# ppwwyyxx/OpenPano

Measured on NVIDIA H100. Metric: Mpixels/sec SIFT+match+blend, higher is better.
Workload: dtype f32

## Files before the change

openpano_b200/csrc/blend.cu:

```cuda
#include "common.cuh"
#include "blur_tile.cuh"
#include <math.h>
#include <string.h>
#include <vector>
#include <algorithm>
#include <climits>
#include <memory>

struct BlendImg {
  union {
    const float* rgb;
    const unsigned char* pix;
  };
  int w, h;
  int x0, y0, x1, y1;
  double hi[9];
  long long roi_off;
  long long plane;
  long long mask_off;
  int rw, rh, pitch;
  int channels;
};

template <class Src> __device__ __forceinline__ Src blend_src(const BlendImg& im, const float* lut);
template <> __device__ __forceinline__ SrcF32 blend_src<SrcF32>(const BlendImg& im, const float*) { return SrcF32{im.rgb}; }
template <> __device__ __forceinline__ SrcRgb8 blend_src<SrcRgb8>(const BlendImg& im, const float* lut) {
  return SrcRgb8{im.pix, lut, im.channels};
}
template <> __device__ __forceinline__ SrcPix8 blend_src<SrcPix8>(const BlendImg& im, const float* lut) {
  return SrcPix8{im.pix, lut, im.channels, (size_t)im.w * im.h};
}

struct BlendGeom {
  int projection;
  double res_x, res_y, min_x, min_y;
  const double* col_sin;
  const double* col_cos;
  const double* row_tan;
};

__device__ __forceinline__ void coor_func(const BlendImg& im, const BlendGeom& g, int tx, int ty, double* ox, double* oy) {
  double cx = (double)tx * g.res_x + g.min_x;
  double cy = (double)ty * g.res_y + g.min_y;
  double hx, hy, hz;
  if (g.projection == PANO_PROJ_FLAT) { hx = cx; hy = cy; hz = 1.0; }
  else if (g.projection == PANO_PROJ_CYLINDRICAL) { hx = g.col_sin[tx]; hy = cy; hz = g.col_cos[tx]; }
  else { hx = g.col_sin[tx]; hy = g.row_tan[ty]; hz = g.col_cos[tx]; }
  double rx = im.hi[0] * hx + im.hi[1] * hy + im.hi[2] * hz;
  double ry = im.hi[3] * hx + im.hi[4] * hy + im.hi[5] * hz;
  double rz = im.hi[6] * hx + im.hi[7] * hy + im.hi[8] * hz;
  if (rz < 0) { *ox = -10; *oy = -10; return; }
  double denom = 1.0 / rz;
  *ox = rx * denom + im.w * 0.5;
  *oy = ry * denom + im.h * 0.5;
}

#define TILE_LIST_CAP 64
struct TileList { int n; unsigned short idx[TILE_LIST_CAP]; };

__device__ __forceinline__ void build_tile_list(const BlendImg* __restrict__ imgs, int n, int j0, int i0, int j1, int i1,
                                                TileList* tl) {
  const int tid = threadIdx.y * blockDim.x + threadIdx.x;
  if (tid < 32) {
    int cnt = 0;
    for (int base = 0; base < n; base += 32) {
      const int k = base + tid;
      bool hit = false;
      if (k < n) {
        const BlendImg& im = imgs[k];
        hit = im.y0 <= i1 && im.y1 >= i0 && im.x0 <= j1 && im.x1 >= j0;
      }
      const unsigned bal = __ballot_sync(0xffffffffu, hit);
      if (hit) {
        const int slot = cnt + __popc(bal & ((1u << tid) - 1));
        if (slot < TILE_LIST_CAP) tl->idx[slot] = (unsigned short)k;
      }
      cnt += __popc(bal);
    }
    if (tid == 0) tl->n = (cnt <= TILE_LIST_CAP && n <= 65535) ? cnt : -1;
  }
  __syncthreads();
}


template <class Src>
__device__ __forceinline__ void linear_add_px(const BlendImg* __restrict__ imgs, int n, const TileList& tl,
                                              const BlendGeom& g, int lazy, int ordered, const float* lut, int i, int j,
                                              float& s0, float& s1, float& s2, float& wsum) {
  const int nl = tl.n < 0 ? n : tl.n;
  for (int q = 0; q < nl; ++q) {
    const BlendImg& im = imgs[tl.n < 0 ? q : (int)tl.idx[q]];
    bool in = lazy ? (i >= im.y0 && i < im.y1 && j >= im.x0 && j < im.x1)
                   : (i >= im.y0 && i <= im.y1 && j >= im.x0 && j <= im.x1);
    if (!in) continue;
    double x, y;
    coor_func(im, g, j, i, &x, &y);
    if (x < 0 || x >= im.w || y < 0 || y >= im.h) continue;
    float r = (float)y, c = (float)x;
    float c0, c1, c2;
    if (!interpolate_rgb(blend_src<Src>(im, lut), im.w, im.h, r, c, &c0, &c1, &c2)) continue;
    if (c0 < 0) continue;
    float w = (float)(0.5 - fabs((double)(c / (float)im.w) - 0.5));
    if (!ordered) w = (float)((double)w * (0.5 - fabs((double)(r / (float)im.h) - 0.5)));
    s0 += c0 * w; s1 += c1 * w; s2 += c2 * w;
    wsum += w;
  }
}

__device__ __forceinline__ void linear_resolve_px(int lazy, float s0, float s1, float s2, float wsum, float* p) {
  if (lazy) {
    if (wsum != 0.f) { p[0] = s0 / wsum; p[1] = s1 / wsum; p[2] = s2 / wsum; }
    else { p[0] = -1.f; p[1] = -1.f; p[2] = -1.f; }
  } else {
    if (wsum > 0) {
      float inv = (float)(1.0 / (double)wsum);
      p[0] = s0 * inv; p[1] = s1 * inv; p[2] = s2 * inv;
    } else { p[0] = -1.f; p[1] = -1.f; p[2] = -1.f; }
  }
}

template <class Src>
__global__ void k_linear_blend(const BlendImg* __restrict__ imgs, int n, BlendGeom g, int lazy, int ordered,
                               float* __restrict__ out, int tw, int row0, int row1) {
  __shared__ TileList tl;
  __shared__ float lut[Src::kLut ? 256 : 1];
  if constexpr (Src::kLut) build_rgb8_lut(lut, threadIdx.y * blockDim.x + threadIdx.x);
  {
    const int tj0 = blockIdx.x * blockDim.x, ti0 = row0 + blockIdx.y * blockDim.y;
    build_tile_list(imgs, n, tj0, ti0, tj0 + blockDim.x - 1, ti0 + blockDim.y - 1, &tl);
  }
  int j = blockIdx.x * blockDim.x + threadIdx.x;
  int i = row0 + blockIdx.y * blockDim.y + threadIdx.y;
  if (j >= tw || i >= row1) return;
  float s0 = 0.f, s1 = 0.f, s2 = 0.f, wsum = 0.f;
  linear_add_px<Src>(imgs, n, tl, g, lazy, ordered, lut, i, j, s0, s1, s2, wsum);
  linear_resolve_px(lazy, s0, s1, s2, wsum, out + ((size_t)(i - row0) * tw + j) * 3);
}

template <class Src>
__global__ void k_linear_accumulate(const BlendImg* __restrict__ imgs, int n, BlendGeom g, int lazy, int ordered,
                                    float* __restrict__ sum, float* __restrict__ wsum, int tw, int rx0, int ry0, int rx1,
                                    int ry1) {
  __shared__ TileList tl;
  __shared__ float lut[Src::kLut ? 256 : 1];
  if constexpr (Src::kLut) build_rgb8_lut(lut, threadIdx.y * blockDim.x + threadIdx.x);
  const int tj0 = rx0 + blockIdx.x * blockDim.x, ti0 = ry0 + blockIdx.y * blockDim.y;
  build_tile_list(imgs, n, tj0, ti0, tj0 + blockDim.x - 1, ti0 + blockDim.y - 1, &tl);
  const int j = tj0 + threadIdx.x, i = ti0 + threadIdx.y;
  if (tl.n == 0 || j >= rx1 || i >= ry1) return;
  const size_t t = (size_t)i * tw + j;
  float* p = sum + t * 3;
  float s0 = p[0], s1 = p[1], s2 = p[2], ws = wsum[t];
  linear_add_px<Src>(imgs, n, tl, g, lazy, ordered, lut, i, j, s0, s1, s2, ws);
  p[0] = s0; p[1] = s1; p[2] = s2;
  wsum[t] = ws;
}

__global__ void k_linear_resolve(const float* sum, const float* __restrict__ wsum, float* out, size_t n_px, int lazy) {
  const size_t t = (size_t)blockIdx.x * blockDim.x + threadIdx.x;
  if (t >= n_px) return;
  const float* p = sum + t * 3;
  linear_resolve_px(lazy, p[0], p[1], p[2], wsum[t], out + t * 3);
}

template <class Src>
__global__ void k_mb_first_level(const BlendImg* __restrict__ imgs, BlendGeom g, float* __restrict__ cur,
                                 unsigned char* __restrict__ mask) {
  __shared__ float lut[Src::kLut ? 256 : 1];
  if constexpr (Src::kLut) {
    build_rgb8_lut(lut, threadIdx.y * blockDim.x + threadIdx.x);
    __syncthreads();
  }
  const BlendImg& im = imgs[blockIdx.z];
  int j = blockIdx.x * blockDim.x + threadIdx.x;
  int i = blockIdx.y * blockDim.y + threadIdx.y;
  if (j >= im.rw || i >= im.rh) return;
  double x, y;
  coor_func(im, g, j + im.x0, i + im.y0, &x, &y);
  float c0, c1, c2;
  bool ok = interpolate_rgb(blend_src<Src>(im, lut), im.w, im.h, (float)y, (float)x, &c0, &c1, &c2);
  if (ok && fminf(c0, fminf(c1, c2)) < 0) ok = false;
  const size_t o = (size_t)i * im.pitch + j;
  float* p = cur + im.roi_off + o;
  float ww = 0.f;
  if (!ok) { c0 = 0.f; c1 = 0.f; c2 = 0.f; }
  else {
    double ox = x / im.w - 0.5, oy = y / im.h - 0.5;
    double wd = (0.5 - fabs(ox)) * (0.5 - fabs(oy));
    if (wd < 0.0) wd = 0.0;
    ww = (float)(wd + 1e-6);
  }
  p[0] = c0; p[im.plane] = c1; p[2 * im.plane] = c2; p[3 * im.plane] = ww;
  mask[im.mask_off + o] = ok ? 0 : 1;
}

__global__ void k_mb_weight_argmax(const BlendImg* __restrict__ imgs, int n, float* __restrict__ cur, int tw,
                                   int row0, int row1) {
  __shared__ TileList tl;
  {
    const int tj0 = blockIdx.x * blockDim.x, ti0 = row0 + blockIdx.y * blockDim.y;
    build_tile_list(imgs, n, tj0, ti0, tj0 + blockDim.x - 1, ti0 + blockDim.y - 1, &tl);
  }
  int j = blockIdx.x * blockDim.x + threadIdx.x;
  int i = row0 + blockIdx.y * blockDim.y + threadIdx.y;
  if (j >= tw || i >= row1) return;
  const int nl = tl.n < 0 ? n : tl.n;
  float mx = 0.f;
  int best = -1;
  for (int q = 0; q < nl; ++q) {
    const BlendImg& im = imgs[tl.n < 0 ? q : (int)tl.idx[q]];
    if (i >= im.y0 && i <= im.y1 && j >= im.x0 && j <= im.x1) {
      const float w = __ldg(cur + im.roi_off + 3 * im.plane + (size_t)(i - im.y0) * im.pitch + (j - im.x0));
      if (w > mx) { mx = w; best = q; }
    }
  }
  for (int q = 0; q < nl; ++q) {
    const BlendImg& im = imgs[tl.n < 0 ? q : (int)tl.idx[q]];
    if (i >= im.y0 && i <= im.y1 && j >= im.x0 && j <= im.x1)
      cur[im.roi_off + 3 * im.plane + (size_t)(i - im.y0) * im.pitch + (j - im.x0)] = q == best ? 1.f : 0.f;
  }
}

struct BlurTaps { int center; float taps[64]; };
struct MbPlane { long long off; int w, h, pitch, pad; };

template <int C>
__global__ void __launch_bounds__(BT_THREADS, 4)
k_mb_blur_tma(const MbPlane* __restrict__ planes, const int2* __restrict__ span, int n_planes, int n_tiles,
              const TmaDesc* __restrict__ maps, float* __restrict__ dst, const __grid_constant__ BlurTaps bt) {
  extern __shared__ __align__(128) float smem[];
  __shared__ __align__(8) uint64_t s_bar[2];
  __shared__ BlurTile s_tile[2];
  constexpr int RX = (C + 3) & ~3;
  constexpr int GW = BT_W + 2 * RX, GH = BT_H + 2 * C;
  constexpr int GSZ = (GH * GW + 31) & ~31;
  float* grey0 = smem;
  float* colbuf = smem + 2 * GSZ;
  float* outT = colbuf + BLUR_COLBUF_FLOATS(C);
// ... 134 lines not shown
  if (is_last && touched) {
    v0 = v0 < 1.0f ? v0 : 1.0f; v0 = v0 > 0.f ? v0 : 0.f;
    v1 = v1 < 1.0f ? v1 : 1.0f; v1 = v1 > 0.f ? v1 : 0.f;
    v2 = v2 < 1.0f ? v2 : 1.0f; v2 = v2 > 0.f ? v2 : 0.f;
    dirty = true;
  }
  if (dirty) { p[0] = v0; p[1] = v1; p[2] = v2; }
  if (first || touched) tmask[t] = touched ? 1 : 0;
}

__global__ void k_fill(float* __restrict__ p, size_t n, float v) {
  size_t i = (size_t)blockIdx.x * blockDim.x + threadIdx.x;
  if (i < n) p[i] = v;
}


struct BlendJob {
  std::vector<BlendImg> imgs;
  BlendGeom g;
  int tw = 0, th = 0;
  long long roi_floats = 0;
  long long mask_bytes = 0;
  int max_rw = 0, max_rh = 0;
  std::vector<BlurTaps> level_taps;
  int halo = 0;
  bool strip = false;
  int clip0 = INT_MIN, clip1 = INT_MAX;
  std::vector<double> tab;
  size_t ncol = 0, nrow = 0;
};

struct BlendDev {
  DevBuf<BlendImg> d_imgs;
  DevBuf<double> d_tab;
  DevBuf<float> d_cur, d_next;
  DevBuf<unsigned char> d_mask, d_tmask;
  DevBuf<MbPlane> d_planes;
  DevBuf<int2> d_span;
  DevBuf<TmaDesc> d_maps;
  std::vector<int> centers;
  int n_planes = 0, n_tiles = 0;
  int wrow0 = 0, wrow1 = 0;
};

template <int C>
static cudaError_t launch_mb_blur_tma(pano_ctx* ctx, int grid, const MbPlane* planes, const int2* span, int n_planes,
                                      int n_tiles, const TmaDesc* maps, float* dst, const BlurTaps& bt) {
  constexpr int RX = (C + 3) & ~3, GW = BT_W + 2 * RX, GH = BT_H + 2 * C, GSZ = (GH * GW + 31) & ~31;
  const size_t smem = (size_t)(2 * GSZ + BLUR_COLBUF_FLOATS(C) + BT_H * (BT_W + 1)) * sizeof(float);
  cudaError_t e = cudaFuncSetAttribute(k_mb_blur_tma<C>, cudaFuncAttributeMaxDynamicSharedMemorySize, (int)smem);
  if (e != cudaSuccess) return e;
  k_mb_blur_tma<C><<<grid, BT_THREADS, smem, ctx->stream>>>(planes, span, n_planes, n_tiles, maps, dst, bt);
  return cudaGetLastError();
}

static int blend_plan(pano_ctx* ctx, int n, const pano_blend_image* imgs, const pano_blend_geom* g, int bands,
                      const pano_params* p, int ow, int oh, int row0, int row1, bool need_src, BlendJob* job,
                      const unsigned char* const* pix = nullptr, const int* channels = nullptr) {
  for (int level = 0; level + 1 < bands; ++level) {
    float sigma = (float)(sqrt(level * 2 + 1.0) * 4);
    BlurTaps bt;
    memset(&bt, 0, sizeof(bt));
    int kw = host_gauss_kernel(sigma, p->gauss_window_factor, bt.taps, 63);
    if (kw < 0) return ctx_fail(ctx, PANO_ERR_INVALID, "blend: gaussian window %d too wide", -kw);
    bt.center = kw / 2;
    job->halo += bt.center;
    job->level_taps.push_back(bt);
  }
  job->strip = bands > 0 && (row0 != 0 || row1 != oh);
  job->clip0 = (job->strip && row0 > 0) ? std::max(0, row0 - job->halo) : INT_MIN;
  job->clip1 = (job->strip && row1 < oh) ? row1 + job->halo - 1 : INT_MAX;
  job->imgs.reserve(n);
  for (int k = 0; k < n; ++k) {
    const pano_blend_image& s = imgs[k];
    if ((need_src && !s.rgb_hwc) || s.w < 2 || s.h < 2 || s.x1 < s.x0 || s.y1 < s.y0 || s.x0 < 0 || s.y0 < 0)
      return ctx_fail(ctx, PANO_ERR_INVALID, "blend: image %d has an invalid shape or range", k);
    if (pix && !pix[k]) return ctx_fail(ctx, PANO_ERR_INVALID, "blend: image %d has no pixels", k);
    if (pix)
      if (int rc = pix8_check(ctx, "blend", k, channels[k], pix[k])) return rc;
    job->tw = std::max(job->tw, s.x1); job->th = std::max(job->th, s.y1);
    BlendImg d;
    memset(&d, 0, sizeof(d));
    d.rgb = s.rgb_hwc; d.w = s.w; d.h = s.h;
    if (pix) d.pix = pix[k];
    d.x0 = s.x0; d.x1 = s.x1;
    d.y0 = std::max(s.y0, job->clip0); d.y1 = std::min(s.y1, job->clip1);
    if (d.y0 > d.y1) continue;
    memcpy(d.hi, s.homo_inv, sizeof(d.hi));
    d.rw = d.x1 - d.x0 + 1; d.rh = d.y1 - d.y0 + 1;
    d.pitch = (int)align_up((size_t)d.rw, 32);
    d.plane = (long long)d.pitch * d.rh;
    d.roi_off = job->roi_floats;
    d.mask_off = job->mask_bytes;
    d.channels = pix ? channels[k] : 3;
    job->roi_floats += 4 * d.plane;
    job->mask_bytes += d.plane;
    job->max_rw = std::max(job->max_rw, d.rw); job->max_rh = std::max(job->max_rh, d.rh);
    job->imgs.push_back(d);
  }
  if (job->tw != ow || job->th != oh || ow <= 0 || oh <= 0)
    return ctx_fail(ctx, PANO_ERR_INVALID, "blend: output is %dx%d but target_size is %dx%d", ow, oh, job->tw, job->th);
  if (job->imgs.empty()) return PANO_OK;
  job->ncol = (size_t)job->tw + 2; job->nrow = (size_t)job->th + 2;
  if (g->projection != PANO_PROJ_FLAT) {
    job->tab.resize(2 * job->ncol + job->nrow);
    for (size_t j = 0; j < job->ncol; ++j) {
      double cx = (double)j * g->res_x + g->proj_min_x;
      job->tab[j] = sin(cx); job->tab[job->ncol + j] = cos(cx);
    }
    for (size_t i = 0; i < job->nrow; ++i) {
      double cy = (double)i * g->res_y + g->proj_min_y;
      job->tab[2 * job->ncol + i] = tan(cy);
    }
  }
  job->g.projection = g->projection; job->g.res_x = g->res_x; job->g.res_y = g->res_y;
  job->g.min_x = g->proj_min_x; job->g.min_y = g->proj_min_y;
  return PANO_OK;
}

static int blend_dev_setup(pano_ctx* ctx, BlendJob* job, int bands, int row0, int row1, BlendDev* d) {
  const int n = (int)job->imgs.size(), tw = job->tw, th = job->th;
  int rc = 0;
  if ((rc = d->d_imgs.alloc(ctx, n))) return rc;
  if ((rc = d->d_tab.alloc(ctx, std::max<size_t>(job->tab.size(), 1)))) return rc;
  {
    void* dsts[2] = {d->d_imgs, d->d_tab};
    const void* srcs[2] = {job->imgs.data(), job->tab.data()};
    size_t sizes[2] = {n * sizeof(BlendImg), job->tab.size() * sizeof(double)};
    if ((rc = ctx_put_many(ctx, 2, dsts, srcs, sizes))) return rc;
  }
  job->g.col_sin = d->d_tab; job->g.col_cos = d->d_tab + job->ncol; job->g.row_tan = d->d_tab + 2 * job->ncol;
  if (bands == 0) return PANO_OK;
  const size_t roi = (size_t)job->roi_floats;
  if ((rc = d->d_cur.alloc(ctx, roi))) return rc;
  if ((rc = d->d_next.alloc(ctx, roi))) return rc;
  if ((rc = d->d_mask.alloc(ctx, (size_t)job->mask_bytes))) return rc;
  const size_t strip_px = (size_t)tw * (row1 - row0);
  d->wrow0 = std::max(0, std::max(row0 - job->halo, job->clip0));
  d->wrow1 = std::min(th, job->strip ? row1 + job->halo : th);
  if ((rc = d->d_tmask.alloc(ctx, strip_px))) return rc;
  d->n_planes = 4 * n;
  std::vector<MbPlane> planes(d->n_planes);
  std::vector<int2> span(d->n_planes);
  for (int k = 0; k < n; ++k)
    for (int ch = 0; ch < 4; ++ch) {
      const BlendImg& im = job->imgs[k];
      planes[4 * k + ch] = MbPlane{im.roi_off + ch * im.plane, im.rw, im.rh, im.pitch, 0};
      span[4 * k + ch] = make_int2(d->n_tiles, ceil_div(im.rw, BT_W));
      d->n_tiles += ceil_div(im.rw, BT_W) * ceil_div(im.rh, BT_H);
    }
  if (bands > 1) {
    if ((rc = d->d_planes.alloc(ctx, d->n_planes))) return rc;
    if ((rc = d->d_span.alloc(ctx, d->n_planes))) return rc;
    if ((rc = ctx_put(ctx, d->d_planes, planes.data(), d->n_planes * sizeof(MbPlane)))) return rc;
    if ((rc = ctx_put(ctx, d->d_span, span.data(), d->n_planes * sizeof(int2)))) return rc;
  }
  for (auto& bt : job->level_taps)
    if ((bt.center == 6 || bt.center == 9) && std::find(d->centers.begin(), d->centers.end(), bt.center) == d->centers.end())
      d->centers.push_back(bt.center);
  if (!d->centers.empty()) {
    std::vector<TmaDesc> maps((size_t)d->centers.size() * 2 * d->n_planes);
    for (size_t ci = 0; ci < d->centers.size(); ++ci)
      for (int buf = 0; buf < 2; ++buf)
        for (int q = 0; q < d->n_planes; ++q) {
          const MbPlane& pl = planes[q];
          const int C = d->centers[ci];
          unsigned long long dims[2] = {(unsigned long long)pl.w, (unsigned long long)pl.h};
          unsigned long long strides[1] = {(unsigned long long)pl.pitch * sizeof(float)};
          unsigned box[2] = {(unsigned)(BT_W + 2 * ((C + 3) & ~3)), (unsigned)(BT_H + 2 * C)};
          if ((rc = ctx_tma_encode(ctx, &maps[(ci * 2 + buf) * d->n_planes + q], (buf ? d->d_next : d->d_cur) + pl.off, 2,
                                   dims, strides, box)))
            return rc;
        }
    if ((rc = d->d_maps.alloc(ctx, maps.size()))) return rc;
    if ((rc = ctx_put(ctx, d->d_maps, maps.data(), maps.size() * sizeof(TmaDesc)))) return rc;
  }
  return PANO_OK;
}

static int mb_levels(pano_ctx* ctx, const BlendJob& job, BlendDev* d, int bands, float* d_out, int row0, int row1) {
  const int n = (int)job.imgs.size(), tw = job.tw;
  const dim3 b(32, 8);
  dim3 gw(ceil_div(tw, 32), ceil_div(d->wrow1 - d->wrow0, 8)), gs(ceil_div(tw, 32), ceil_div(row1 - row0, 8));
  PANO_LAUNCH(ctx, "k_mb_weight_argmax", k_mb_weight_argmax, gw, b, 0, d->d_imgs, n, d->d_cur, tw, d->wrow0, d->wrow1);
  float *cur = d->d_cur, *next = d->d_next;
  int buf = 0;
  for (int level = 0; level < bands; ++level) {
    int is_last = level == bands - 1;
    if (!is_last) {
      const BlurTaps& bt = job.level_taps[level];
      const int c = bt.center;
      cudaError_t e = cudaSuccess;
      ctx->launches++;
      if (ctx->profiling) ctx_prof_begin(ctx, "k_mb_blur");
      auto ci = std::find(d->centers.begin(), d->centers.end(), c);
      if (ci != d->centers.end()) {
        const TmaDesc* maps = d->d_maps + ((size_t)(ci - d->centers.begin()) * 2 + buf) * d->n_planes;
        const int grid = std::min(d->n_tiles, ctx->num_sms * 4);
        e = c == 6 ? launch_mb_blur_tma<6>(ctx, grid, d->d_planes, d->d_span, d->n_planes, d->n_tiles, maps, next, bt)
                   : launch_mb_blur_tma<9>(ctx, grid, d->d_planes, d->d_span, d->n_planes, d->n_tiles, maps, next, bt);
      } else {
        const size_t smem = sizeof(float) * ((size_t)(MB_TH + 2 * c) * (MB_TW + 2 * c) + (size_t)MB_TH * (MB_TW + 2 * c));
        if (smem > 200 * 1024) {
          if (ctx->profiling) ctx_prof_end(ctx);
          return ctx_fail(ctx, PANO_ERR_INVALID, "blend: gaussian window %d too wide", 2 * c + 1);
        }
        e = cudaFuncSetAttribute(k_mb_blur_generic, cudaFuncAttributeMaxDynamicSharedMemorySize, (int)smem);
        if (e == cudaSuccess) {
          k_mb_blur_generic<<<d->n_tiles, 256, smem, ctx->stream>>>(d->d_planes, d->d_span, d->n_planes, cur, next, bt);
          e = cudaGetLastError();
        }
      }
      if (ctx->profiling) ctx_prof_end(ctx);
      if (e != cudaSuccess) return ctx_cuda(ctx, e, "k_mb_blur");
    }
    PANO_LAUNCH(ctx, "k_mb_accumulate", k_mb_accumulate, gs, b, 0, d->d_imgs, n, cur, next, d->d_mask, level == 0 ? 1 : 0,
              is_last, d_out, d->d_tmask, tw, row0, row1);
    if (!is_last) { std::swap(cur, next); buf ^= 1; }
  }
  return PANO_OK;
}

template <class Src>
static int blend_run(pano_ctx* ctx, const BlendJob& job, BlendDev* d, int bands, const pano_params* p, float* d_out,
                     int row0, int row1) {
  const int n = (int)job.imgs.size(), tw = job.tw;
  const dim3 b(32, 8);
  constexpr bool pix8 = std::is_same<Src, SrcPix8>::value;
  if (bands == 0) {
    dim3 gs(ceil_div(tw, 32), ceil_div(row1 - row0, 8));
    PANO_LAUNCH(ctx, pix8 ? "k_linear_blend_pix8" : Src::kLut ? "k_linear_blend_rgb8" : "k_linear_blend",
                k_linear_blend<Src>, gs, b, 0, d->d_imgs, n, job.g, p->lazy_read, p->ordered_input, d_out, tw, row0, row1);
    return PANO_OK;
  }
  dim3 gr(ceil_div(job.max_rw, 32), ceil_div(job.max_rh, 8), n);
  PANO_LAUNCH(ctx, pix8 ? "k_mb_first_level_pix8" : "k_mb_first_level", k_mb_first_level<Src>, gr, b, 0, d->d_imgs, job.g,
              d->d_cur, d->d_mask);
  return mb_levels(ctx, job, d, bands, d_out, row0, row1);
}

static int blend_device(pano_ctx* ctx, int n, const pano_blend_image* imgs, const pano_blend_geom* g, int bands,
                        const pano_params* p, float* d_out, int ow, int oh, int row0, int row1,
                        const unsigned char* const* pix = nullptr, const int* channels = nullptr) {
  if (!ctx || n <= 0 || !imgs || !g || !p || !d_out || bands < 0) return PANO_ERR_INVALID;
  if (n > PANO_MAX_IMAGES)
    return ctx_fail(ctx, PANO_ERR_INVALID, "blend: %d images (limit %d)", n, PANO_MAX_IMAGES);
  if (row0 < 0 || row1 > oh || row0 > row1)
    return ctx_fail(ctx, PANO_ERR_INVALID, "blend: rows [%d, %d) outside the %d-row canvas", row0, row1, oh);
  if (row0 == row1) return PANO_OK;
  BlendJob job;
  int rc = blend_plan(ctx, n, imgs, g, bands, p, ow, oh, row0, row1, !pix, &job, pix, channels);
  if (rc) return rc;
  if (job.imgs.empty()) {
    size_t nfl = (size_t)job.tw * (row1 - row0) * 3;
    PANO_LAUNCH(ctx, "k_fill", k_fill, (unsigned)((nfl + 255) / 256), 256, 0, d_out, nfl, -1.f);
    return PANO_OK;
  }
  BlendDev dev;
  if ((rc = blend_dev_setup(ctx, &job, bands, row0, row1, &dev))) return rc;
  if (pix && std::any_of(channels, channels + n, pix8_layout))
    return blend_run<SrcPix8>(ctx, job, &dev, bands, p, d_out, row0, row1);
  return pix ? blend_run<SrcRgb8>(ctx, job, &dev, bands, p, d_out, row0, row1)
             : blend_run<SrcF32>(ctx, job, &dev, bands, p, d_out, row0, row1);
}

struct pano_blend_stream {
  pano_ctx* ctx = nullptr;
  int n = 0, bands = 0, lazy = 0, ordered = 0;
  BlendJob job;
  BlendDev dev;
  DevBuf<float> d_sum;
  DevBuf<float> d_wsum;
  int added = 0, err = 0;
  bool finished = false;
  UploadRing ring;
};

static int stream_fail(pano_blend_stream* s, int rc) { s->err = rc; return rc; }
#define STREAM_MISUSE(s, ...) stream_fail((s), ctx_fail((s)->ctx, PANO_ERR_INVALID, __VA_ARGS__))
#define STREAM_CUDA(s, call)                                               \
  do {                                                                     \
    cudaError_t _e = (call);                                               \
    if (_e != cudaSuccess) return stream_fail((s), ctx_cuda((s)->ctx, _e, #call)); \
  } while (0)

static int stream_upload(pano_blend_stream* s, int first, int count, const void* const* srcs, bool u8, int channels,
                         BlendImg* win, int* slot_out) {
  std::vector<size_t> bytes(count);
  std::vector<const void*> d_src(count);
  for (int k = 0; k < count; ++k) {
    const BlendImg& im = s->job.imgs[first + k];
    bytes[k] = (size_t)im.w * im.h * (u8 ? (size_t)pix8_bytes(channels) : 3 * sizeof(float));
  }
  if (int rc = s->ring.upload(s->ctx, count, srcs, bytes.data(), d_src.data(), slot_out)) return stream_fail(s, rc);
  for (int k = 0; k < count; ++k) win[k].pix = (const unsigned char*)d_src[k];
  return PANO_OK;
}

template <class Src>
static int stream_launch(pano_blend_stream* s, const BlendImg* d_win, const BlendImg* win, int count) {
  pano_ctx* ctx = s->ctx;
  const BlendJob& job = s->job;
  const dim3 b(32, 8);
  constexpr bool pix8 = std::is_same<Src, SrcPix8>::value;
  if (s->bands == 0) {
    int x0 = INT_MAX, y0 = INT_MAX, x1 = 0, y1 = 0;
    for (int k = 0; k < count; ++k) {
      x0 = std::min(x0, win[k].x0); y0 = std::min(y0, win[k].y0);
      x1 = std::max(x1, win[k].x1 + 1); y1 = std::max(y1, win[k].y1 + 1);
    }
    x1 = std::min(x1, job.tw); y1 = std::min(y1, job.th);
    if (x0 >= x1 || y0 >= y1) return PANO_OK;
    dim3 g(ceil_div(x1 - x0, 32), ceil_div(y1 - y0, 8));
    PANO_LAUNCH(ctx, pix8 ? "k_linear_accumulate_pix8" : "k_linear_accumulate", k_linear_accumulate<Src>, g, b, 0, d_win,
                count, job.g, s->lazy, s->ordered, s->d_sum, s->d_wsum, job.tw, x0, y0, x1, y1);
  } else {
    int rw = 0, rh = 0;
    for (int k = 0; k < count; ++k) { rw = std::max(rw, win[k].rw); rh = std::max(rh, win[k].rh); }
    dim3 g(ceil_div(rw, 32), ceil_div(rh, 8), count);
    PANO_LAUNCH(ctx, pix8 ? "k_mb_first_level_pix8" : "k_mb_first_level", k_mb_first_level<Src>, g, b, 0, d_win, job.g,
                s->dev.d_cur, s->dev.d_mask);
  }
  return PANO_OK;
}

static int stream_resolve(pano_blend_stream* s, float* d_out) {
  pano_ctx* ctx = s->ctx;
  if (s->bands > 0) return mb_levels(ctx, s->job, &s->dev, s->bands, d_out, 0, s->job.th);
  const size_t npx = (size_t)s->job.tw * s->job.th;
  PANO_LAUNCH(ctx, "k_linear_resolve", k_linear_resolve, (unsigned)((npx + 255) / 256), 256, 0, s->d_sum, s->d_wsum,
              d_out, npx, s->lazy);
  return PANO_OK;
}

static int stream_finish_check(pano_blend_stream* s, const void* out) {
  if (s->err) return s->err;
  if (!out) return STREAM_MISUSE(s, "blend stream: null output");
  if (s->finished) return STREAM_MISUSE(s, "blend stream: already finished");
  if (s->added != s->n) return STREAM_MISUSE(s, "blend stream: finish after %d of %d images", s->added, s->n);
  s->finished = true;
  return PANO_OK;
}

extern "C" {

int pano_blend_target_size(int n, const pano_blend_image* imgs, int* ow, int* oh) {
  if (n <= 0 || !imgs || !ow || !oh) return PANO_ERR_INVALID;
  int tw = 0, th = 0;
  for (int k = 0; k < n; ++k) { tw = std::max(tw, imgs[k].x1); th = std::max(th, imgs[k].y1); }
  *ow = tw; *oh = th;
  return PANO_OK;
}

int pano_blend_dev(pano_ctx* ctx, int n, const pano_blend_image* imgs, const pano_blend_geom* g, int bands,
                   const pano_params* p, float* d_out, int ow, int oh) {
  ctx_enter(ctx);
  return blend_device(ctx, n, imgs, g, bands, p, d_out, ow, oh, 0, oh);
}

int pano_blend_rgb8_dev(pano_ctx* ctx, int n, const pano_blend_image* imgs, const unsigned char* const* d_pix,
                        const int* channels, const pano_blend_geom* g, int bands, const pano_params* p, float* d_out,
                        int ow, int oh) {
  ctx_enter(ctx);
  if (!ctx) return PANO_ERR_INVALID;
  if (!d_pix || !channels) return ctx_fail(ctx, PANO_ERR_INVALID, "blend rgb8: null source list");
  return blend_device(ctx, n, imgs, g, bands, p, d_out, ow, oh, 0, oh, d_pix, channels);
}

int pano_blend_rows_dev(pano_ctx* ctx, int n, const pano_blend_image* imgs, const pano_blend_geom* g, int bands,
                        const pano_params* p, float* d_out_rows, int ow, int oh, int row0, int row1) {
  ctx_enter(ctx);
  return blend_device(ctx, n, imgs, g, bands, p, d_out_rows, ow, oh, row0, row1);
}

int pano_blend_rows_rgb8_dev(pano_ctx* ctx, int n, const pano_blend_image* imgs, const unsigned char* const* d_pix,
                             const int* channels, const pano_blend_geom* g, int bands, const pano_params* p,
                             float* d_out_rows, int ow, int oh, int row0, int row1) {
  ctx_enter(ctx);
  if (!ctx) return PANO_ERR_INVALID;
  if (!d_pix || !channels) return ctx_fail(ctx, PANO_ERR_INVALID, "blend rows rgb8: null source list");
  return blend_device(ctx, n, imgs, g, bands, p, d_out_rows, ow, oh, row0, row1, d_pix, channels);
}

int pano_blend_stream_create(pano_ctx* ctx, int n, const pano_blend_image* imgs, const pano_blend_geom* g, int bands,
                             const pano_params* p, int ow, int oh, pano_blend_stream** out) {
  ctx_enter(ctx);
  if (!ctx || !out) return PANO_ERR_INVALID;
  *out = nullptr;
  if (n <= 0 || !imgs || !g || !p || bands < 0) return ctx_fail(ctx, PANO_ERR_INVALID, "blend stream: bad argument");
  if (n > PANO_MAX_IMAGES)
    return ctx_fail(ctx, PANO_ERR_INVALID, "blend stream: %d images (limit %d)", n, PANO_MAX_IMAGES);
  std::unique_ptr<pano_blend_stream> s(new pano_blend_stream);
  s->ctx = ctx; s->n = n; s->bands = bands; s->lazy = p->lazy_read; s->ordered = p->ordered_input;
  int rc = blend_plan(ctx, n, imgs, g, bands, p, ow, oh, 0, oh, false, &s->job);
  if (!rc) rc = blend_dev_setup(ctx, &s->job, bands, 0, oh, &s->dev);
  if (rc) return rc;
// ... 108 lines not shown
```

openpano_b200/csrc/common.cuh:

```cuda
#pragma once

#include <cuda_runtime.h>
#include <stdint.h>
#include <string>
#include <vector>
#include <map>
#include <memory>
#include <type_traits>
#include <unordered_map>

#include "../../include/pano_b200.h"


int  ctx_alloc(pano_ctx* ctx, void** p, size_t bytes);
void ctx_cache_release(pano_ctx* ctx, size_t keep_bytes);
void ctx_free(pano_ctx* ctx, void* p);
template <class T>
class DevBuf {
 public:
  DevBuf() = default;
  DevBuf(pano_ctx* ctx, T* p) : ctx_(ctx), p_(p) {}
  DevBuf(const DevBuf&) = delete;
  DevBuf& operator=(const DevBuf&) = delete;
  DevBuf(DevBuf&& o) noexcept : ctx_(o.ctx_), p_(o.release()) {}
// ... 288 lines not shown
  float m = absx > absy ? absx : absy;
  if ((double)m < 1e-6) return (float)(-PANO_PI);
  float a = (absy < absx ? absy : absx) / m;
  float s = a * a;
  double sd = (double)s, ad = (double)a;
  float r = (float)(((-0.0464964749 * sd + 0.15931422) * sd - 0.327622764) * sd * ad + ad);
  if (absy > absx) r = (float)(PANO_PI_2 - (double)r);
  if (x < 0) r = (float)(PANO_PI - (double)r);
  if (y < 0) r = -r;
  return r;
}

__device__ __forceinline__ void mag_ort_at(const float* __restrict__ img, int w, int x, int y,
                                           float* mag, float* ort) {
  const float* row = img + (size_t)y * w;
  float dy = row[x + w] - row[x - w];
  float dx = row[x + 1] - row[x - 1];
  *mag = glibc_hypotf(dx, dy);
  *ort = (float)((double)fast_atan(dy, dx) + PANO_PI);
}

struct SrcF32 {
  const float* img;
  static constexpr bool kMayBeNo = true, kLut = false;
  __device__ __forceinline__ void fetch(int w, int fr, int fc, float* q) const {
    const float* p00 = img + ((size_t)fr * w + fc) * 3;
    const float* p10 = p00 + (size_t)w * 3;
#pragma unroll
    for (int k = 0; k < 6; ++k) { q[k] = __ldg(p00 + k); q[6 + k] = __ldg(p10 + k); }
  }
};
struct SrcRgb8 {
  const unsigned char* pix;
  const float* lut;
  int channels;
  static constexpr bool kMayBeNo = false, kLut = true;
  __device__ __forceinline__ void fetch(int w, int fr, int fc, float* q) const {
    if (channels == 1) {
      const unsigned char* p00 = pix + (size_t)fr * w + fc;
      const float a = (float)__ldg(p00), b = (float)__ldg(p00 + 1);
      const float c = (float)__ldg(p00 + w), d = (float)__ldg(p00 + w + 1);
      q[0] = q[1] = q[2] = a; q[3] = q[4] = q[5] = b;
      q[6] = q[7] = q[8] = c; q[9] = q[10] = q[11] = d;
    } else {
      const unsigned char* p00 = pix + ((size_t)fr * w + fc) * 3;
      const unsigned char* p10 = p00 + (size_t)w * 3;
#pragma unroll
      for (int k = 0; k < 6; ++k) { q[k] = lut[__ldg(p00 + k)]; q[6 + k] = lut[__ldg(p10 + k)]; }
    }
  }
};
struct SrcPix8 {
  const unsigned char* pix;
  const float* lut;
  int fmt;
  size_t plane;
  static constexpr bool kMayBeNo = false, kLut = true;
  __device__ __forceinline__ void fetch(int w, int fr, int fc, float* q) const {
    if (fmt == PANO_PIX_RGBA) {
      const unsigned* p00 = reinterpret_cast<const unsigned*>(pix) + (size_t)fr * w + fc;
      const unsigned t[4] = {__ldg(p00), __ldg(p00 + 1), __ldg(p00 + w), __ldg(p00 + w + 1)};
#pragma unroll
      for (int k = 0; k < 4; ++k) {
        q[3 * k] = lut[t[k] & 0xff]; q[3 * k + 1] = lut[(t[k] >> 8) & 0xff]; q[3 * k + 2] = lut[(t[k] >> 16) & 0xff];
      }
    } else if (fmt == PANO_PIX_RGB_PLANAR) {
      const unsigned char* p00 = pix + (size_t)fr * w + fc;
#pragma unroll
      for (int ch = 0; ch < 3; ++ch) {
        const unsigned char* p = p00 + ch * plane;
        q[ch] = lut[__ldg(p)]; q[3 + ch] = lut[__ldg(p + 1)];
        q[6 + ch] = lut[__ldg(p + w)]; q[9 + ch] = lut[__ldg(p + w + 1)];
      }
    } else {
      SrcRgb8{pix, lut, fmt}.fetch(w, fr, fc, q);
    }
  }
};
__device__ __forceinline__ void build_rgb8_lut(float* lut, int tid) {
  if (tid < 256) lut[tid] = (float)((double)tid / 255.0);
}

template <class Src>
__device__ __forceinline__ bool interpolate_rgb(const Src& src, int w, int h, float r, float c, float* o0, float* o1,
                                                float* o2) {
  int fr = (int)floorf(r), fc = (int)floorf(c);
  if (fr < 0 || fc < 0 || fc + 1 >= w || fr + 1 >= h) return false;
  r -= (float)fr;
  c -= (float)fc;
  float q[12];
  src.fetch(w, fr, fc, q);
  const float q00 = q[0], q01 = q[1], q02 = q[2], q03 = q[3], q04 = q[4], q05 = q[5];
  const float q10 = q[6], q11 = q[7], q12 = q[8], q13 = q[9], q14 = q[10], q15 = q[11];
  if (Src::kMayBeNo && (q00 < 0 || q10 < 0 || q13 < 0 || q03 < 0)) return false;
  float w00 = (1 - r) * (1 - c), w10 = r * (1 - c), w11 = r * c, w01 = (1 - r) * c;
  float a0 = 0.f + q00 * w00, a1 = 0.f + q01 * w00, a2 = 0.f + q02 * w00;
  a0 += q10 * w10; a1 += q11 * w10; a2 += q12 * w10;
  a0 += q13 * w11; a1 += q14 * w11; a2 += q15 * w11;
  a0 += q03 * w01; a1 += q04 * w01; a2 += q05 * w01;
  *o0 = a0; *o1 = a1; *o2 = a2;
  return true;
}
__device__ __forceinline__ bool interpolate_rgb(const float* __restrict__ img, int w, int h, float r, float c,
                                                float* o0, float* o1, float* o2) {
  return interpolate_rgb(SrcF32{img}, w, h, r, c, o0, o1, o2);
}

#endif
```

Measured before the change: 11380.

## Restructure linear blend to warp-ballot image culling with hoisted per-column mapping

Replaces the shared-memory per-block tile list with per-warp ballot culling over images, so each warp iterates only over images overlapping its 32xLB_ROWS strip and no block-wide sync is needed. The homography mapping is split into column-dependent and row-dependent partial products, which allows reuse across rows. Image metadata is loaded with 16-byte vector loads, and width and height are precomputed as doubles. Launch bounds are added to raise occupancy. The costs are more redundant header loads per warp and possible register pressure from the forced minimum block counts.

Measured after the change: 11540 (median of 6 runs). About the same (+1.4%).

```diff
diff --git a/openpano_b200/csrc/blend.cu b/openpano_b200/csrc/blend.cu
--- a/openpano_b200/csrc/blend.cu
+++ b/openpano_b200/csrc/blend.cu
@@ -5,6 +5,7 @@
 #include <vector>
 #include <algorithm>
 #include <climits>
+#include <cstddef>
 #include <memory>
 
 struct BlendImg {
@@ -20,7 +21,10 @@
   long long mask_off;
   int rw, rh, pitch;
   int channels;
+  double wd, hd;
 };
+static_assert(offsetof(BlendImg, x0) % 16 == 0 && offsetof(BlendImg, hi) % 16 == 0 && offsetof(BlendImg, wd) % 16 == 0 &&
+                  sizeof(BlendImg) % 16 == 0, "BlendImg: the linear kernels load these fields as 16-byte vectors");
 
 template <class Src> __device__ __forceinline__ Src blend_src(const BlendImg& im, const float* lut);
 template <> __device__ __forceinline__ SrcF32 blend_src<SrcF32>(const BlendImg& im, const float*) { return SrcF32{im.rgb}; }
@@ -39,6 +43,30 @@
   const double* row_tan;
 };
 
+struct MapCol { double x0, x2, y0, y2, z0, z2; };
+struct MapRow { double x1, y1, z1; };
+
+__device__ __forceinline__ void map_col_axes(const BlendGeom& g, int tx, double* hx, double* hz) {
+  if (g.projection == PANO_PROJ_FLAT) { *hx = (double)tx * g.res_x + g.min_x; *hz = 1.0; }
+  else { *hx = g.col_sin[tx]; *hz = g.col_cos[tx]; }
+}
+__device__ __forceinline__ double map_row_axis(const BlendGeom& g, int ty) {
+  if (g.projection == PANO_PROJ_FLAT || g.projection == PANO_PROJ_CYLINDRICAL) return (double)ty * g.res_y + g.min_y;
+  return g.row_tan[ty];
+}
+__device__ __forceinline__ MapCol map_col(const double* hi, double hx, double hz) {
+  return MapCol{hi[0] * hx, hi[2] * hz, hi[3] * hx, hi[5] * hz, hi[6] * hx, hi[8] * hz};
+}
+__device__ __forceinline__ MapRow map_row(const double* hi, double hy) { return MapRow{hi[1] * hy, hi[4] * hy, hi[7] * hy}; }
+__device__ __forceinline__ void map_px(const MapCol& c, const MapRow& r, double hw, double hh, double* ox, double* oy) {
+  const double rx = c.x0 + r.x1 + c.x2;
+  const double ry = c.y0 + r.y1 + c.y2;
+  const double rz = c.z0 + r.z1 + c.z2;
+  if (rz < 0) { *ox = -10; *oy = -10; return; }
+  const double denom = 1.0 / rz;
+  *ox = rx * denom + hw;
+  *oy = ry * denom + hh;
+}
 __device__ __forceinline__ void coor_func(const BlendImg& im, const BlendGeom& g, int tx, int ty, double* ox, double* oy) {
   double cx = (double)tx * g.res_x + g.min_x;
   double cy = (double)ty * g.res_y + g.min_y;
@@ -82,28 +110,71 @@
   __syncthreads();
 }
 
+#ifndef LB_ROWS
+#define LB_ROWS 1
+#endif
+#define LB_TH (8 * LB_ROWS)
+template <class Src> constexpr int lb_min_ctas() { return std::is_same<Src, SrcPix8>::value ? 5 : 6; }
+
+__device__ __forceinline__ unsigned strip_hits(const BlendImg* __restrict__ imgs, int n, int base, int jw0, int iw0) {
+  const int k = base + (int)threadIdx.x;
+  bool hit = false;
+  if (k < n) {
+    const BlendImg& im = imgs[k];
+    hit = im.y0 <= iw0 + LB_ROWS - 1 && im.y1 >= iw0 && im.x0 <= jw0 + 31 && im.x1 >= jw0;
+  }
+  return __ballot_sync(0xffffffffu, hit);
+}
 
 template <class Src>
-__device__ __forceinline__ void linear_add_px(const BlendImg* __restrict__ imgs, int n, const TileList& tl,
-                                              const BlendGeom& g, int lazy, int ordered, const float* lut, int i, int j,
-                                              float& s0, float& s1, float& s2, float& wsum) {
-  const int nl = tl.n < 0 ? n : tl.n;
-  for (int q = 0; q < nl; ++q) {
-    const BlendImg& im = imgs[tl.n < 0 ? q : (int)tl.idx[q]];
-    bool in = lazy ? (i >= im.y0 && i < im.y1 && j >= im.x0 && j < im.x1)
-                   : (i >= im.y0 && i <= im.y1 && j >= im.x0 && j <= im.x1);
-    if (!in) continue;
-    double x, y;
-    coor_func(im, g, j, i, &x, &y);
-    if (x < 0 || x >= im.w || y < 0 || y >= im.h) continue;
-    float r = (float)y, c = (float)x;
-    float c0, c1, c2;
-    if (!interpolate_rgb(blend_src<Src>(im, lut), im.w, im.h, r, c, &c0, &c1, &c2)) continue;
-    if (c0 < 0) continue;
-    float w = (float)(0.5 - fabs((double)(c / (float)im.w) - 0.5));
-    if (!ordered) w = (float)((double)w * (0.5 - fabs((double)(r / (float)im.h) - 0.5)));
-    s0 += c0 * w; s1 += c1 * w; s2 += c2 * w;
-    wsum += w;
+__device__ __forceinline__ void linear_add_strip(const BlendImg* __restrict__ imgs, int n, const BlendGeom& g, int lazy,
+                                                 int ordered, const float* lut, int jw0, int iw0, int j1, int i1,
+                                                 float (&s)[LB_ROWS][4]) {
+  const int j = jw0 + (int)threadIdx.x;
+  const bool col_ok = j < j1;
+  double hx = 0.0, hz = 0.0, hy[LB_ROWS];
+  if (col_ok) map_col_axes(g, j, &hx, &hz);
+#pragma unroll
+  for (int r = 0; r < LB_ROWS; ++r) hy[r] = iw0 + r < i1 ? map_row_axis(g, iw0 + r) : 0.0;
+  for (int base = 0; base < n; base += 32) {
+    for (unsigned m = strip_hits(imgs, n, base, jw0, iw0); m; m &= m - 1) {
+      const BlendImg* im = imgs + base + __ffs(m) - 1;
+      const int4 roi = __ldg(reinterpret_cast<const int4*>(&im->x0));
+      const int2 wh = __ldg(reinterpret_cast<const int2*>(&im->w));
+      const double2 wdh = __ldg(reinterpret_cast<const double2*>(&im->wd));
+      double hi[9];
+#pragma unroll
+      for (int e = 0; e < 8; e += 2) {
+        const double2 v = __ldg(reinterpret_cast<const double2*>(im->hi + e));
+        hi[e] = v.x; hi[e + 1] = v.y;
+      }
+      hi[8] = __ldg(im->hi + 8);
+      const Src src = blend_src<Src>(*im, lut);
+      if (!col_ok || !(j >= roi.x && (lazy ? j < roi.z : j <= roi.z))) continue;
+      const int w = wh.x, h = wh.y;
+      const MapCol mc = map_col(hi, hx, hz);
+#pragma unroll
+      for (int r = 0; r < LB_ROWS; ++r) {
+        const int i = iw0 + r;
+        if (!(i < i1 && i >= roi.y && (lazy ? i < roi.w : i <= roi.w))) continue;
+        double x, y;
+        map_px(mc, map_row(hi, hy[r]), wdh.x * 0.5, wdh.y * 0.5, &x, &y);
+        if (x < 0 || x >= wdh.x || y < 0 || y >= wdh.y) continue;
+        const float rv = (float)y, cv = (float)x;
+        const int fr = (int)floorf(rv), fc = (int)floorf(cv);
+        if (fr < 0 || fc < 0 || fc + 1 >= w || fr + 1 >= h) continue;
+        float q[12];
+        src.fetch(w, fr, fc, q);
+        const bool no = Src::kMayBeNo && (q[0] < 0 || q[6] < 0 || q[9] < 0 || q[3] < 0);
+        float c0, c1, c2;
+        interp_blend<SrcRgb8>(q, rv - (float)fr, cv - (float)fc, &c0, &c1, &c2);
+        if (no || c0 < 0) continue;
+        float wv = (float)(0.5 - fabs((double)(cv / (float)w) - 0.5));
+        if (!ordered) wv = (float)((double)wv * (0.5 - fabs((double)(rv / (float)h) - 0.5)));
+        s[r][0] += c0 * wv; s[r][1] += c1 * wv; s[r][2] += c2 * wv;
+        s[r][3] += wv;
+      }
+    }
   }
 }
 
@@ -120,40 +191,58 @@
 }
 
 template <class Src>
-__global__ void k_linear_blend(const BlendImg* __restrict__ imgs, int n, BlendGeom g, int lazy, int ordered,
-                               float* __restrict__ out, int tw, int row0, int row1) {
-  __shared__ TileList tl;
+__global__ void __launch_bounds__(256, lb_min_ctas<Src>()) k_linear_blend(const BlendImg* __restrict__ imgs, int n, BlendGeom g, int lazy,
+                                                      int ordered, float* __restrict__ out, int tw, int row0, int row1) {
   __shared__ float lut[Src::kLut ? 256 : 1];
-  if constexpr (Src::kLut) build_rgb8_lut(lut, threadIdx.y * blockDim.x + threadIdx.x);
-  {
-    const int tj0 = blockIdx.x * blockDim.x, ti0 = row0 + blockIdx.y * blockDim.y;
-    build_tile_list(imgs, n, tj0, ti0, tj0 + blockDim.x - 1, ti0 + blockDim.y - 1, &tl);
-  }
-  int j = blockIdx.x * blockDim.x + threadIdx.x;
-  int i = row0 + blockIdx.y * blockDim.y + threadIdx.y;
-  if (j >= tw || i >= row1) return;
-  float s0 = 0.f, s1 = 0.f, s2 = 0.f, wsum = 0.f;
-  linear_add_px<Src>(imgs, n, tl, g, lazy, ordered, lut, i, j, s0, s1, s2, wsum);
-  linear_resolve_px(lazy, s0, s1, s2, wsum, out + ((size_t)(i - row0) * tw + j) * 3);
+  if constexpr (Src::kLut) {
+    build_rgb8_lut(lut, threadIdx.y * blockDim.x + threadIdx.x);
+    __syncthreads();
+  }
+  const int jw0 = blockIdx.x * 32, iw0 = row0 + blockIdx.y * LB_TH + threadIdx.y * LB_ROWS;
+  float s[LB_ROWS][4] = {};
+  linear_add_strip<Src>(imgs, n, g, lazy, ordered, lut, jw0, iw0, tw, row1, s);
+  const int j = jw0 + threadIdx.x;
+  if (j >= tw) return;
+#pragma unroll
+  for (int r = 0; r < LB_ROWS; ++r) {
+    const int i = iw0 + r;
+    if (i < row1) linear_resolve_px(lazy, s[r][0], s[r][1], s[r][2], s[r][3], out + ((size_t)(i - row0) * tw + j) * 3);
+  }
 }
 
 template <class Src>
-__global__ void k_linear_accumulate(const BlendImg* __restrict__ imgs, int n, BlendGeom g, int lazy, int ordered,
-                                    float* __restrict__ sum, float* __restrict__ wsum, int tw, int rx0, int ry0, int rx1,
-                                    int ry1) {
-  __shared__ TileList tl;
+__global__ void __launch_bounds__(256) k_linear_accumulate(const BlendImg* __restrict__ imgs, int n, BlendGeom g,
+                                                           int lazy, int ordered, float* __restrict__ sum,
+                                                           float* __restrict__ wsum, int tw, int rx0, int ry0, int rx1,
+                                                           int ry1) {
   __shared__ float lut[Src::kLut ? 256 : 1];
-  if constexpr (Src::kLut) build_rgb8_lut(lut, threadIdx.y * blockDim.x + threadIdx.x);
-  const int tj0 = rx0 + blockIdx.x * blockDim.x, ti0 = ry0 + blockIdx.y * blockDim.y;
-  build_tile_list(imgs, n, tj0, ti0, tj0 + blockDim.x - 1, ti0 + blockDim.y - 1, &tl);
-  const int j = tj0 + threadIdx.x, i = ti0 + threadIdx.y;
-  if (tl.n == 0 || j >= rx1 || i >= ry1) return;
-  const size_t t = (size_t)i * tw + j;
-  float* p = sum + t * 3;
-  float s0 = p[0], s1 = p[1], s2 = p[2], ws = wsum[t];
-  linear_add_px<Src>(imgs, n, tl, g, lazy, ordered, lut, i, j, s0, s1, s2, ws);
-  p[0] = s0; p[1] = s1; p[2] = s2;
-  wsum[t] = ws;
+  if constexpr (Src::kLut) {
+    build_rgb8_lut(lut, threadIdx.y * blockDim.x + threadIdx.x);
+    __syncthreads();
+  }
+  const int jw0 = rx0 + blockIdx.x * 32, iw0 = ry0 + blockIdx.y * LB_TH + threadIdx.y * LB_ROWS;
+  unsigned any = 0;
+  for (int base = 0; base < n && !any; base += 32) any = strip_hits(imgs, n, base, jw0, iw0);
+  if (!any) return;
+  const int j = jw0 + threadIdx.x;
+  float s[LB_ROWS][4] = {};
+#pragma unroll
+  for (int r = 0; r < LB_ROWS; ++r) {
+    const int i = iw0 + r;
+    if (j < rx1 && i < ry1) {
+      const size_t t = (size_t)i * tw + j;
+      s[r][0] = sum[t * 3]; s[r][1] = sum[t * 3 + 1]; s[r][2] = sum[t * 3 + 2]; s[r][3] = wsum[t];
+    }
+  }
+  linear_add_strip<Src>(imgs, n, g, lazy, ordered, lut, jw0, iw0, rx1, ry1, s);
+#pragma unroll
+  for (int r = 0; r < LB_ROWS; ++r) {
+    const int i = iw0 + r;
+    if (j < rx1 && i < ry1) {
+      const size_t t = (size_t)i * tw + j;
+      sum[t * 3] = s[r][0]; sum[t * 3 + 1] = s[r][1]; sum[t * 3 + 2] = s[r][2]; wsum[t] = s[r][3];
+    }
+  }
 }
 
 __global__ void k_linear_resolve(const float* sum, const float* __restrict__ wsum, float* out, size_t n_px, int lazy) {
@@ -454,6 +543,7 @@
     BlendImg d;
     memset(&d, 0, sizeof(d));
     d.rgb = s.rgb_hwc; d.w = s.w; d.h = s.h;
+    d.wd = s.w; d.hd = s.h;
     if (pix) d.pix = pix[k];
     d.x0 = s.x0; d.x1 = s.x1;
     d.y0 = std::max(s.y0, job->clip0); d.y1 = std::min(s.y1, job->clip1);
@@ -600,7 +690,7 @@
   const dim3 b(32, 8);
   constexpr bool pix8 = std::is_same<Src, SrcPix8>::value;
   if (bands == 0) {
-    dim3 gs(ceil_div(tw, 32), ceil_div(row1 - row0, 8));
+    dim3 gs(ceil_div(tw, 32), ceil_div(row1 - row0, LB_TH));
     PANO_LAUNCH(ctx, pix8 ? "k_linear_blend_pix8" : Src::kLut ? "k_linear_blend_rgb8" : "k_linear_blend",
                 k_linear_blend<Src>, gs, b, 0, d->d_imgs, n, job.g, p->lazy_read, p->ordered_input, d_out, tw, row0, row1);
     return PANO_OK;
@@ -683,7 +773,7 @@
     }
     x1 = std::min(x1, job.tw); y1 = std::min(y1, job.th);
     if (x0 >= x1 || y0 >= y1) return PANO_OK;
-    dim3 g(ceil_div(x1 - x0, 32), ceil_div(y1 - y0, 8));
+    dim3 g(ceil_div(x1 - x0, 32), ceil_div(y1 - y0, LB_TH));
     PANO_LAUNCH(ctx, pix8 ? "k_linear_accumulate_pix8" : "k_linear_accumulate", k_linear_accumulate<Src>, g, b, 0, d_win,
                 count, job.g, s->lazy, s->ordered, s->d_sum, s->d_wsum, job.tw, x0, y0, x1, y1);
   } else {
diff --git a/openpano_b200/csrc/common.cuh b/openpano_b200/csrc/common.cuh
--- a/openpano_b200/csrc/common.cuh
+++ b/openpano_b200/csrc/common.cuh
@@ -394,14 +394,7 @@
 }
 
 template <class Src>
-__device__ __forceinline__ bool interpolate_rgb(const Src& src, int w, int h, float r, float c, float* o0, float* o1,
-                                                float* o2) {
-  int fr = (int)floorf(r), fc = (int)floorf(c);
-  if (fr < 0 || fc < 0 || fc + 1 >= w || fr + 1 >= h) return false;
-  r -= (float)fr;
-  c -= (float)fc;
-  float q[12];
-  src.fetch(w, fr, fc, q);
+__device__ __forceinline__ bool interp_blend(const float* q, float r, float c, float* o0, float* o1, float* o2) {
   const float q00 = q[0], q01 = q[1], q02 = q[2], q03 = q[3], q04 = q[4], q05 = q[5];
   const float q10 = q[6], q11 = q[7], q12 = q[8], q13 = q[9], q14 = q[10], q15 = q[11];
   if (Src::kMayBeNo && (q00 < 0 || q10 < 0 || q13 < 0 || q03 < 0)) return false;
@@ -413,6 +406,17 @@
   *o0 = a0; *o1 = a1; *o2 = a2;
   return true;
 }
+template <class Src>
+__device__ __forceinline__ bool interpolate_rgb(const Src& src, int w, int h, float r, float c, float* o0, float* o1,
+                                                float* o2) {
+  int fr = (int)floorf(r), fc = (int)floorf(c);
+  if (fr < 0 || fc < 0 || fc + 1 >= w || fr + 1 >= h) return false;
+  r -= (float)fr;
+  c -= (float)fc;
+  float q[12];
+  src.fetch(w, fr, fc, q);
+  return interp_blend<Src>(q, r, c, o0, o1, o2);
+}
 __device__ __forceinline__ bool interpolate_rgb(const float* __restrict__ img, int w, int h, float r, float c,
                                                 float* o0, float* o1, float* o2) {
   return interpolate_rgb(SrcF32{img}, w, h, r, c, o0, o1, o2);
```
